# robin-karlsson0/ViT-Adapter

Hardware: AMD Instinct MI355X
Metric: images/sec ViT-Adapter-B 1024x1024 fwd+bwd (+AdamW step) (higher is better)
Workload: dtype bf16; 1 GPU; ViT-Adapter-base_det (det) 1024x1024, per-GPU batch 2, train mode, drop_path 0.3, SyncBN, step = fwd+bwd+AdamW; global_batch=2, parallelism=dp1, hip_graph=True, rccl_ranks=1, gemm_candidates_rejected=0

## Files before the change

vit-adapter_amd/csrc/attn_win.hip:

```cpp
#include "attn_common.h"
#include "common.h"

namespace vah {
namespace attn {
namespace {



template <typename T, int NB, int NT>
__device__ __forceinline__ void stage_rows(const T *const (&src)[NT], const int64_t (&lds)[NT], T *const (&dst)[NT],
                                           const RowMap &rm, int z, int N) {
    vec8<T> x[4][NT];
    bool ok[4];
#pragma unroll
    for (int it = 0; it < 4; ++it) {
        const int i = threadIdx.x + it * 64 * NB;
        const int row = i >> 3, c = (i & 7) * 8;
        const int64_t g = row < N ? grow(rm, z, row, N) : -1;
        ok[it] = g >= 0;
        const int64_t gl = ok[it] ? g : 0;
#pragma unroll
        for (int t = 0; t < NT; ++t) x[it][t] = *reinterpret_cast<const vec8<T> *>(src[t] + gl * lds[t] + c);
    }
#pragma unroll
    for (int it = 0; it < 4; ++it) {
        const int i = threadIdx.x + it * 64 * NB;
        const int row = i >> 3, c = (i & 7) * 8;
#pragma unroll
        for (int t = 0; t < NT; ++t) {
            vec8<T> y = x[it][t];
#pragma unroll
            for (int j = 0; j < 8; ++j) y[j] = ok[it] ? y[j] : (T)0.f;
            *reinterpret_cast<vec8<T> *>(dst[t] + row * kPadRow + c) = y;
        }
    }
}

template <typename T>
__device__ __forceinline__ const T *tile_lane_base(const T *tile, int lane) {
    const int grp = lane >> 4, i16 = lane & 15;
    return tile + (4 * (grp >> 1) + (i16 >> 2)) * kPadRow + 16 * (grp & 1) + 4 * (i16 & 3);
}
template <typename T>
__device__ __forceinline__ vec8<T> load_tr(const T *base, int tok0, int db) {
    const T *p0 = base + tok0 * kPadRow + 32 * db;
    return tr_frag<T>(p0, p0 + 8 * kPadRow);
}

template <typename T, int NB>
__global__ __launch_bounds__(64 * NB) __attribute__((amdgpu_waves_per_eu((2 * NB + 3) / 4, (2 * NB + 3) / 4))) void attn_win_fwd_kernel(
    const T *__restrict__ q, const T *__restrict__ k, const T *__restrict__ v, int64_t ld, RowMap rm,
    int N, int H, float scale_log2, T *__restrict__ out, int64_t ld_out, float *__restrict__ lse) {
    constexpr int ROWS = 32 * NB;
    __shared__ __attribute__((aligned(16))) T s_k[ROWS * kPadRow];
    __shared__ __attribute__((aligned(16))) T s_v[ROWS * kPadRow];
    const int h = blockIdx.x, z = blockIdx.y;
    const int wave = threadIdx.x >> 6, lane = threadIdx.x & 63;
    const int r = lane & 31, hf = lane >> 5;
    const T *qb = q + (int64_t)h * kHD, *kb_ = k + (int64_t)h * kHD, *vb = v + (int64_t)h * kHD;

    const int qrow = wave * 32 + r;
    const int64_t gq = qrow < N ? grow(rm, z, qrow, N) : -1;
    vec8<T> qf[4];
    {
        const int64_t gl = gq >= 0 ? gq : 0;
#pragma unroll
        for (int kk = 0; kk < 4; ++kk) {
            const vec8<T> x = *reinterpret_cast<const vec8<T> *>(qb + gl * ld + 16 * kk + 8 * hf);
#pragma unroll
            for (int j = 0; j < 8; ++j) qf[kk][j] = gq >= 0 ? x[j] : (T)0.f;
        }
    }
    stage_rows<T, NB, 2>({kb_, vb}, {ld, ld}, {s_k, s_v}, rm, z, N);
    __syncthreads();

    auto s_block = [&](int kb) {
        f32x16 s = zero16();
#pragma unroll
        for (int kk = 0; kk < 4; ++kk)
            s = mfma(*reinterpret_cast<const vec8<T> *>(s_k + (kb * 32 + r) * kPadRow + 16 * kk + 8 * hf), qf[kk], s);
        if (kb == NB - 1) {
#pragma unroll
            for (int i = 0; i < 16; ++i)
                if (kb * 32 + crow(i, hf) >= N) s[i] = -INFINITY;
        }
        return s;
    };
    float mx = -INFINITY;
#pragma unroll 1
    for (int kb = 0; kb < NB; ++kb) {
        const f32x16 s = s_block(kb);
#pragma unroll
        for (int i = 0; i < 16; ++i) mx = fmaxf(mx, s[i]);
    }
    mx = fmaxf(mx, __shfl_xor(mx, 32, 64));
    const float m = mx * scale_log2;

    f32x16 o[2] = {zero16(), zero16()};
    float psum = 0.f;
    const T *vbase = tile_lane_base(s_v, lane);
#pragma unroll 1
    for (int kb = 0; kb < NB; ++kb) {
        f32x16 s = s_block(kb);
#pragma unroll
        for (int i = 0; i < 16; ++i) {
            s[i] = __builtin_amdgcn_exp2f(s[i] * scale_log2 - m);
            psum += s[i];
        }
#pragma unroll
        for (int sp = 0; sp < 2; ++sp) {
            const vec8<T> pf = pack_half<T>(s, sp);
#pragma unroll
            for (int db = 0; db < 2; ++db) o[db] = mfma(load_tr(vbase, kb * 32 + 16 * sp, db), pf, o[db]);
        }
    }
    const float l_tot = psum + __shfl_xor(psum, 32, 64);

    const float inv = 1.f / l_tot;
    if (qrow < N && gq >= 0) {
        T *op = out + gq * ld_out + (int64_t)h * kHD;
#pragma unroll
        for (int db = 0; db < 2; ++db)
#pragma unroll
            for (int g = 0; g < 4; ++g) {
                vec4<T> w;
#pragma unroll
                for (int j = 0; j < 4; ++j) w[j] = (T)(o[db][4 * g + j] * inv);
                *reinterpret_cast<vec4<T> *>(op + db * 32 + 8 * g + 4 * hf) = w;
            }
        if (hf == 0) lse[((int64_t)z * H + h) * N + qrow] = m + log2f(l_tot);
    } else if (qrow < N && hf == 0) {
        lse[((int64_t)z * H + h) * N + qrow] = INFINITY;
    }
}


template <typename T, int NB>
__global__ __launch_bounds__(64 * NB) void attn_win_bwd_kernel(
    const T *__restrict__ q, const T *__restrict__ k, const T *__restrict__ v, int64_t ld,
    const T *__restrict__ o, const T *__restrict__ d_o, int64_t ld_out, RowMap rm, const float *__restrict__ lse,
    int N, int H, float scale, float scale_log2, T *__restrict__ dq, T *__restrict__ dk, T *__restrict__ dv,
    int64_t ld_d) {
    constexpr int ROWS = 32 * NB;
    extern __shared__ __attribute__((aligned(16))) unsigned char smem[];
    T *s_q = reinterpret_cast<T *>(smem);
    T *s_k = s_q + ROWS * kPadRow, *s_v = s_k + ROWS * kPadRow, *s_do = s_v + ROWS * kPadRow;
    float *s_lse = reinterpret_cast<float *>(s_do + ROWS * kPadRow), *s_delta = s_lse + ROWS;
    const int h = blockIdx.x, z = blockIdx.y;
    const int wave = threadIdx.x >> 6, lane = threadIdx.x & 63;
    const int r = lane & 31, hf = lane >> 5;
    const int row = wave * 32 + r;
    const int64_t grow_ = row < N ? grow(rm, z, row, N) : -1;
    const bool stored = grow_ >= 0;

    float part = 0.f;
    {
        const int64_t gl = stored ? grow_ : 0;
        const T *op = o + gl * ld_out + (int64_t)h * kHD + 32 * hf, *gp = d_o + gl * ld_out + (int64_t)h * kHD + 32 * hf;
        vec8<T> a[4], b[4];
#pragma unroll
        for (int c = 0; c < 4; ++c) {
            a[c] = *reinterpret_cast<const vec8<T> *>(op + 8 * c);
            b[c] = *reinterpret_cast<const vec8<T> *>(gp + 8 * c);
        }
#pragma unroll
        for (int c = 0; c < 4; ++c)
#pragma unroll
            for (int j = 0; j < 8; ++j) part += (float)a[c][j] * (float)b[c][j];
    }
    const float lse_raw = lse[((int64_t)z * H + h) * N + (row < N ? row : 0)];
    stage_rows<T, NB, 4>({q + (int64_t)h * kHD, k + (int64_t)h * kHD, v + (int64_t)h * kHD, d_o + (int64_t)h * kHD},
                      {ld, ld, ld, ld_out}, {s_q, s_k, s_v, s_do}, rm, z, N);
    const float delta_q = stored ? part + __shfl_xor(part, 32, 64) : 0.f;
    const float lse_q = stored ? lse_raw : INFINITY;
    if (hf == 0) {
        s_lse[row] = lse_q;
        s_delta[row] = delta_q;
    }
    __syncthreads();

    {
        vec8<T> qf[4], dof[4];
#pragma unroll
        for (int kk = 0; kk < 4; ++kk) {
            qf[kk] = *reinterpret_cast<const vec8<T> *>(s_q + row * kPadRow + 16 * kk + 8 * hf);
            dof[kk] = *reinterpret_cast<const vec8<T> *>(s_do + row * kPadRow + 16 * kk + 8 * hf);
        }
        f32x16 acc[2] = {zero16(), zero16()};
        const T *kbase = tile_lane_base(s_k, lane);
#pragma unroll
        for (int j = 0; j < NB; ++j) {
            f32x16 s = zero16(), dp = zero16();
#pragma unroll
            for (int kk = 0; kk < 4; ++kk) {
                const vec8<T> ak = *reinterpret_cast<const vec8<T> *>(s_k + (j * 32 + r) * kPadRow + 16 * kk + 8 * hf);
                const vec8<T> av = *reinterpret_cast<const vec8<T> *>(s_v + (j * 32 + r) * kPadRow + 16 * kk + 8 * hf);
                s = mfma(ak, qf[kk], s);
                dp = mfma(av, dof[kk], dp);
            }
#pragma unroll
            for (int i = 0; i < 16; ++i) s[i] = __builtin_amdgcn_exp2f(s[i] * scale_log2 - lse_q) * (dp[i] - delta_q);
#pragma unroll
            for (int sp = 0; sp < 2; ++sp) {
                const vec8<T> pf = pack_half<T>(s, sp);
#pragma unroll
                for (int db = 0; db < 2; ++db) acc[db] = mfma(load_tr(kbase, j * 32 + 16 * sp, db), pf, acc[db]);
            }
        }
        if (stored) {
            T *op = dq + grow_ * ld_d + (int64_t)h * kHD;
#pragma unroll
            for (int db = 0; db < 2; ++db)
#pragma unroll
                for (int g = 0; g < 4; ++g) {
                    vec4<T> w;
#pragma unroll
                    for (int jj = 0; jj < 4; ++jj) w[jj] = (T)(acc[db][4 * g + jj] * scale);
                    *reinterpret_cast<vec4<T> *>(op + db * 32 + 8 * g + 4 * hf) = w;
                }
        }
    }

    {
        vec8<T> kf[4], vf[4];
#pragma unroll
        for (int kk = 0; kk < 4; ++kk) {
            kf[kk] = *reinterpret_cast<const vec8<T> *>(s_k + row * kPadRow + 16 * kk + 8 * hf);
            vf[kk] = *reinterpret_cast<const vec8<T> *>(s_v + row * kPadRow + 16 * kk + 8 * hf);
        }
        f32x16 dkt[2] = {zero16(), zero16()}, dvt[2] = {zero16(), zero16()};
        const T *qbase = tile_lane_base(s_q, lane), *dobase = tile_lane_base(s_do, lane);
#pragma unroll 1
        for (int i = 0; i < NB; ++i) {
            f32x16 s = zero16(), dp = zero16();
#pragma unroll
            for (int kk = 0; kk < 4; ++kk) {
                const vec8<T> aq = *reinterpret_cast<const vec8<T> *>(s_q + (i * 32 + r) * kPadRow + 16 * kk + 8 * hf);
                const vec8<T> ad = *reinterpret_cast<const vec8<T> *>(s_do + (i * 32 + r) * kPadRow + 16 * kk + 8 * hf);
                s = mfma(aq, kf[kk], s);
                dp = mfma(ad, vf[kk], dp);
            }
#pragma unroll
            for (int g = 0; g < 4; ++g) {
                const float4 l4 = *reinterpret_cast<const float4 *>(s_lse + i * 32 + 8 * g + 4 * hf);
                const float4 d4 = *reinterpret_cast<const float4 *>(s_delta + i * 32 + 8 * g + 4 * hf);
                const float ls[4] = {l4.x, l4.y, l4.z, l4.w}, de[4] = {d4.x, d4.y, d4.z, d4.w};
#pragma unroll
                for (int jj = 0; jj < 4; ++jj) {
                    const int e = 4 * g + jj;
                    const float p = __builtin_amdgcn_exp2f(s[e] * scale_log2 - ls[jj]);
                    s[e] = p;
                    dp[e] = p * (dp[e] - de[jj]);
                }
            }
#pragma unroll
            for (int sp = 0; sp < 2; ++sp) {
                const vec8<T> pf = pack_half<T>(s, sp), dsf = pack_half<T>(dp, sp);
#pragma unroll
                for (int db = 0; db < 2; ++db) {
                    dvt[db] = mfma(load_tr(dobase, i * 32 + 16 * sp, db), pf, dvt[db]);
                    dkt[db] = mfma(load_tr(qbase, i * 32 + 16 * sp, db), dsf, dkt[db]);
                }
            }
        }
        if (stored) {
            T *pk = dk + grow_ * ld_d + (int64_t)h * kHD, *pv = dv + grow_ * ld_d + (int64_t)h * kHD;
#pragma unroll
            for (int db = 0; db < 2; ++db)
#pragma unroll
                for (int g = 0; g < 4; ++g) {
                    vec4<T> wk, wv;
#pragma unroll
                    for (int jj = 0; jj < 4; ++jj) {
                        wk[jj] = (T)(dkt[db][4 * g + jj] * scale);
                        wv[jj] = (T)dvt[db][4 * g + jj];
                    }
                    *reinterpret_cast<vec4<T> *>(pk + db * 32 + 8 * g + 4 * hf) = wk;
                    *reinterpret_cast<vec4<T> *>(pv + db * 32 + 8 * g + 4 * hf) = wv;
                }
        }
    }
}

template <typename T, int NB>
int launch_win_bwd(const T *q, const T *k, const T *v, int64_t ld, const T *o, const T *d_o,
                   int64_t ld_out, RowMap rm, const float *lse, int64_t Z, int64_t H, int N, float scale, T *dq,
                   T *dk, T *dv, int64_t ld_d, hipStream_t st) {
    constexpr int lds = 4 * 32 * NB * kPadRow * 2 + 2 * 32 * NB * 4;
    if (int rc = allow_dynamic_lds((const void *)attn_win_bwd_kernel<T, NB>, lds, "attn_win_bwd")) return rc;
    hipLaunchKernelGGL((attn_win_bwd_kernel<T, NB>), dim3((unsigned)H, (unsigned)Z), dim3(64 * NB), lds, st, q, k, v, ld, o, d_o,
                       ld_out, rm, lse, N, (int)H, scale, scale * 1.4426950408889634f, dq, dk, dv, ld_d);
    return check_launch("attn_win_bwd");
}

template <typename T, int NB>
int launch_win_fwd(const T *q, const T *k, const T *v, int64_t ld, RowMap rm, int64_t Z, int64_t H, int N,
                   float scale_log2, T *out, int64_t ld_out, float *lse, hipStream_t st) {
    hipLaunchKernelGGL((attn_win_fwd_kernel<T, NB>), dim3((unsigned)H, (unsigned)Z), dim3(64 * NB), 0, st, q, k, v, ld, rm, N, (int)H,
                       scale_log2, out, ld_out, lse);
    return check_launch("attn_win_fwd");
}

}

template <typename T>
int attn_win_fwd_resident(const void *q, const void *k, const void *v, int64_t ld, RowMap rm, int64_t Z, int64_t H, int64_t N,
                          float scale, void *out, int64_t ld_out, float *lse, hipStream_t st) {
    if (N < 1 || N > 224 || Z > 65535 || H > 65535) return -1;
    const int NB = (int)((N + 31) / 32);
    const float scale_log2 = scale * 1.4426950408889634f;
#define VAH_CASE(B_)                                                                                                    \
    if (NB == B_)                                                                                                       \
        return launch_win_fwd<T, B_>((const T *)q, (const T *)k, (const T *)v, ld, rm, Z, H, (int)N, scale_log2, \
                                  (T *)out, ld_out, lse, st)
    VAH_CASE(1);
    VAH_CASE(2);
    VAH_CASE(3);
    VAH_CASE(4);
    VAH_CASE(5);
    VAH_CASE(6);
    VAH_CASE(7);
#undef VAH_CASE
    return -1;
}


template <typename T>
int attn_win_bwd_resident(const void *q, const void *k, const void *v, int64_t ld, const void *o, const void *d_o,
                          int64_t ld_out, RowMap rm, const float *lse, int64_t Z, int64_t H, int64_t N, float scale, void *dq,
                          void *dk, void *dv, int64_t ld_d, hipStream_t st) {
    if (N < 1 || N > 224 || Z > 65535 || H > 65535) return -1;
    const int NB = (int)((N + 31) / 32);
#define VAH_CASE(B_)                                                                                                     \
    if (NB == B_)                                                                                                        \
        return launch_win_bwd<T, B_>((const T *)q, (const T *)k, (const T *)v, ld, (const T *)o,         \
                                  (const T *)d_o, ld_out, rm, lse, Z, H, (int)N, scale, (T *)dq, (T *)dk, \
                                  (T *)dv, ld_d, st)
    VAH_CASE(1);
    VAH_CASE(2);
    VAH_CASE(3);
    VAH_CASE(4);
    VAH_CASE(5);
    VAH_CASE(6);
    VAH_CASE(7);
#undef VAH_CASE
    return -1;
}

template int attn_win_fwd_resident<__bf16>(const void *, const void *, const void *, int64_t, RowMap, int64_t, int64_t, int64_t, float,
                                           void *, int64_t, float *, hipStream_t);
template int attn_win_fwd_resident<_Float16>(const void *, const void *, const void *, int64_t, RowMap, int64_t, int64_t, int64_t,
                                             float, void *, int64_t, float *, hipStream_t);
template int attn_win_bwd_resident<__bf16>(const void *, const void *, const void *, int64_t, const void *, const void *, int64_t,
                                           RowMap, const float *, int64_t, int64_t, int64_t, float, void *, void *, void *, int64_t,
                                           hipStream_t);
template int attn_win_bwd_resident<_Float16>(const void *, const void *, const void *, int64_t, const void *, const void *, int64_t,
                                             RowMap, const float *, int64_t, int64_t, int64_t, float, void *, void *, void *, int64_t,
                                             hipStream_t);

}
}
```

Baseline: 77.28 images/sec.

## Skip padded rows in windowed attention via per-window-class item mapping

Flattens the grid to one dimension and maps each block to a (window, head) item grouped by window class: interior, bottom edge, right edge and corner. Each block computes the real row count of its window, exits the waves that only cover padding, and loops over real key blocks only. Padded keys that the original code treated as zero-valued keys are accounted for analytically in the softmax denominator, and padded rows get an infinite LSE. This removes the MFMA and load work spent on padding in edge windows, at the cost of extra index arithmetic per block and more complex masking logic.

```diff
diff --git a/vit-adapter_amd/csrc/attn_win.hip b/vit-adapter_amd/csrc/attn_win.hip
--- a/vit-adapter_amd/csrc/attn_win.hip
+++ b/vit-adapter_amd/csrc/attn_win.hip
@@ -7,31 +7,93 @@
 
 
 
+struct WinItem {
+    int z, h;
+    int vw, Nr, win;
+    int W;
+    int64_t row0;
+    __device__ __forceinline__ int64_t grow(int c) const {
+        const int ly = c / vw;
+        return row0 + (int64_t)ly * W + (c - ly * vw);
+    }
+    __device__ __forceinline__ int local(int c) const {
+        const int ly = c / vw;
+        return ly * win + (c - ly * vw);
+    }
+};
+
+__device__ __forceinline__ WinItem win_item(const RowMap &rm, int item, int H, int Z, int N) {
+    WinItem it;
+    if (rm.win == 0) {
+        it.z = item / H;
+        it.h = item - it.z * H;
+        it.vw = it.Nr = it.win = N;
+        it.W = 0;
+        it.row0 = (int64_t)it.z * N;
+        return it;
+    }
+    const int nwy = rm.nwin / rm.nwx, fy = rm.H / rm.win, fx = rm.W / rm.win, B = Z / rm.nwin;
+    const int cnt[4] = {fy * fx, (nwy - fy) * fx, fy * (rm.nwx - fx), (nwy - fy) * (rm.nwx - fx)};
+    int t = item, cls = 0;
+#pragma unroll
+    for (int c = 0; c < 3; ++c)
+        if (cls == c && t >= B * H * cnt[c]) {
+            t -= B * H * cnt[c];
+            cls = c + 1;
+        }
+    const int u = t / H, per = cnt[cls];
+    it.h = t - u * H;
+    const int b = u / per, j = u - b * per;
+    int wy, wx;
+    if (cls == 0) {
+        wy = j / fx;
+        wx = j - wy * fx;
+    } else if (cls == 1) {
+        wy = fy;
+        wx = j;
+    } else if (cls == 2) {
+        wy = j;
+        wx = fx;
+    } else {
+        wy = fy;
+        wx = fx;
+    }
+    it.z = b * rm.nwin + wy * rm.nwx + wx;
+    const int y0 = wy * rm.win, x0 = wx * rm.win;
+    const int vh = min(rm.win, rm.H - y0);
+    it.vw = min(rm.win, rm.W - x0);
+    it.Nr = vh * it.vw;
+    it.win = rm.win;
+    it.W = rm.W;
+    it.row0 = ((int64_t)b * rm.H + y0) * rm.W + x0;
+    return it;
+}
+
 template <typename T, int NB, int NT>
 __device__ __forceinline__ void stage_rows(const T *const (&src)[NT], const int64_t (&lds)[NT], T *const (&dst)[NT],
-                                           const RowMap &rm, int z, int N) {
+                                           const WinItem &wi, int rows) {
     vec8<T> x[4][NT];
-    bool ok[4];
 #pragma unroll
     for (int it = 0; it < 4; ++it) {
         const int i = threadIdx.x + it * 64 * NB;
         const int row = i >> 3, c = (i & 7) * 8;
-        const int64_t g = row < N ? grow(rm, z, row, N) : -1;
-        ok[it] = g >= 0;
-        const int64_t gl = ok[it] ? g : 0;
-#pragma unroll
-        for (int t = 0; t < NT; ++t) x[it][t] = *reinterpret_cast<const vec8<T> *>(src[t] + gl * lds[t] + c);
+#pragma unroll
+        for (int t = 0; t < NT; ++t)
+#pragma unroll
+            for (int j = 0; j < 8; ++j) x[it][t][j] = (T)0.f;
+        if (row < wi.Nr) {
+            const int64_t g = wi.grow(row);
+#pragma unroll
+            for (int t = 0; t < NT; ++t) x[it][t] = *reinterpret_cast<const vec8<T> *>(src[t] + g * lds[t] + c);
+        }
     }
 #pragma unroll
     for (int it = 0; it < 4; ++it) {
         const int i = threadIdx.x + it * 64 * NB;
         const int row = i >> 3, c = (i & 7) * 8;
-#pragma unroll
-        for (int t = 0; t < NT; ++t) {
-            vec8<T> y = x[it][t];
-#pragma unroll
-            for (int j = 0; j < 8; ++j) y[j] = ok[it] ? y[j] : (T)0.f;
-            *reinterpret_cast<vec8<T> *>(dst[t] + row * kPadRow + c) = y;
+        if (row < rows) {
+#pragma unroll
+            for (int t = 0; t < NT; ++t) *reinterpret_cast<vec8<T> *>(dst[t] + row * kPadRow + c) = x[it][t];
         }
     }
 }
@@ -54,41 +116,50 @@
     constexpr int ROWS = 32 * NB;
     __shared__ __attribute__((aligned(16))) T s_k[ROWS * kPadRow];
     __shared__ __attribute__((aligned(16))) T s_v[ROWS * kPadRow];
-    const int h = blockIdx.x, z = blockIdx.y;
+    const WinItem wi = win_item(rm, blockIdx.x, H, gridDim.x / H, N);
+    const int h = wi.h, z = wi.z, Nr = wi.Nr;
+    const int nb = (Nr + 31) >> 5;
+    const int n_pad = N - Nr;
     const int wave = threadIdx.x >> 6, lane = threadIdx.x & 63;
     const int r = lane & 31, hf = lane >> 5;
     const T *qb = q + (int64_t)h * kHD, *kb_ = k + (int64_t)h * kHD, *vb = v + (int64_t)h * kHD;
+    float *lse_w = lse + ((int64_t)z * H + h) * N;
 
     const int qrow = wave * 32 + r;
-    const int64_t gq = qrow < N ? grow(rm, z, qrow, N) : -1;
+    const bool real_q = qrow < Nr;
+    const int64_t gq = real_q ? wi.grow(qrow) : 0;
     vec8<T> qf[4];
-    {
-        const int64_t gl = gq >= 0 ? gq : 0;
-#pragma unroll
-        for (int kk = 0; kk < 4; ++kk) {
-            const vec8<T> x = *reinterpret_cast<const vec8<T> *>(qb + gl * ld + 16 * kk + 8 * hf);
-#pragma unroll
-            for (int j = 0; j < 8; ++j) qf[kk][j] = gq >= 0 ? x[j] : (T)0.f;
-        }
-    }
-    stage_rows<T, NB, 2>({kb_, vb}, {ld, ld}, {s_k, s_v}, rm, z, N);
+#pragma unroll
+    for (int kk = 0; kk < 4; ++kk) {
+#pragma unroll
+        for (int j = 0; j < 8; ++j) qf[kk][j] = (T)0.f;
+        if (real_q) qf[kk] = *reinterpret_cast<const vec8<T> *>(qb + gq * ld + 16 * kk + 8 * hf);
+    }
+    stage_rows<T, NB, 2>({kb_, vb}, {ld, ld}, {s_k, s_v}, wi, nb * 32);
+    if (n_pad > 0) {
+        for (int i = threadIdx.x; i < N; i += 64 * NB) {
+            const int ly = i / wi.win, lx = i - ly * wi.win;
+            if (lx >= wi.vw || ly * wi.vw >= Nr) lse_w[i] = INFINITY;
+        }
+    }
     __syncthreads();
+    if (wave >= nb) return;
 
     auto s_block = [&](int kb) {
         f32x16 s = zero16();
 #pragma unroll
         for (int kk = 0; kk < 4; ++kk)
             s = mfma(*reinterpret_cast<const vec8<T> *>(s_k + (kb * 32 + r) * kPadRow + 16 * kk + 8 * hf), qf[kk], s);
-        if (kb == NB - 1) {
+        if (kb == nb - 1) {
 #pragma unroll
             for (int i = 0; i < 16; ++i)
-                if (kb * 32 + crow(i, hf) >= N) s[i] = -INFINITY;
+                if (kb * 32 + crow(i, hf) >= Nr) s[i] = -INFINITY;
         }
         return s;
     };
-    float mx = -INFINITY;
+    float mx = n_pad > 0 ? 0.f : -INFINITY;
 #pragma unroll 1
-    for (int kb = 0; kb < NB; ++kb) {
+    for (int kb = 0; kb < nb; ++kb) {
         const f32x16 s = s_block(kb);
 #pragma unroll
         for (int i = 0; i < 16; ++i) mx = fmaxf(mx, s[i]);
@@ -100,7 +171,7 @@
     float psum = 0.f;
     const T *vbase = tile_lane_base(s_v, lane);
 #pragma unroll 1
-    for (int kb = 0; kb < NB; ++kb) {
+    for (int kb = 0; kb < nb; ++kb) {
         f32x16 s = s_block(kb);
 #pragma unroll
         for (int i = 0; i < 16; ++i) {
@@ -114,10 +185,11 @@
             for (int db = 0; db < 2; ++db) o[db] = mfma(load_tr(vbase, kb * 32 + 16 * sp, db), pf, o[db]);
         }
     }
-    const float l_tot = psum + __shfl_xor(psum, 32, 64);
+    float l_tot = psum + __shfl_xor(psum, 32, 64);
+    if (n_pad > 0) l_tot += (float)n_pad * __builtin_amdgcn_exp2f(-m);
 
     const float inv = 1.f / l_tot;
-    if (qrow < N && gq >= 0) {
+    if (real_q) {
         T *op = out + gq * ld_out + (int64_t)h * kHD;
 #pragma unroll
         for (int db = 0; db < 2; ++db)
@@ -128,9 +200,7 @@
                 for (int j = 0; j < 4; ++j) w[j] = (T)(o[db][4 * g + j] * inv);
                 *reinterpret_cast<vec4<T> *>(op + db * 32 + 8 * g + 4 * hf) = w;
             }
-        if (hf == 0) lse[((int64_t)z * H + h) * N + qrow] = m + log2f(l_tot);
-    } else if (qrow < N && hf == 0) {
-        lse[((int64_t)z * H + h) * N + qrow] = INFINITY;
+        if (hf == 0) lse_w[wi.local(qrow)] = m + log2f(l_tot);
     }
 }
 
@@ -146,17 +216,18 @@
     T *s_q = reinterpret_cast<T *>(smem);
     T *s_k = s_q + ROWS * kPadRow, *s_v = s_k + ROWS * kPadRow, *s_do = s_v + ROWS * kPadRow;
     float *s_lse = reinterpret_cast<float *>(s_do + ROWS * kPadRow), *s_delta = s_lse + ROWS;
-    const int h = blockIdx.x, z = blockIdx.y;
+    const WinItem wi = win_item(rm, blockIdx.x, H, gridDim.x / H, N);
+    const int h = wi.h, z = wi.z, Nr = wi.Nr;
+    const int nb = (Nr + 31) >> 5;
     const int wave = threadIdx.x >> 6, lane = threadIdx.x & 63;
     const int r = lane & 31, hf = lane >> 5;
     const int row = wave * 32 + r;
-    const int64_t grow_ = row < N ? grow(rm, z, row, N) : -1;
-    const bool stored = grow_ >= 0;
-
-    float part = 0.f;
-    {
-        const int64_t gl = stored ? grow_ : 0;
-        const T *op = o + gl * ld_out + (int64_t)h * kHD + 32 * hf, *gp = d_o + gl * ld_out + (int64_t)h * kHD + 32 * hf;
+    const bool stored = row < Nr;
+    const int64_t grow_ = stored ? wi.grow(row) : 0;
+
+    float part = 0.f, lse_raw = INFINITY;
+    if (stored) {
+        const T *op = o + grow_ * ld_out + (int64_t)h * kHD + 32 * hf, *gp = d_o + grow_ * ld_out + (int64_t)h * kHD + 32 * hf;
         vec8<T> a[4], b[4];
 #pragma unroll
         for (int c = 0; c < 4; ++c) {
@@ -167,17 +238,18 @@
         for (int c = 0; c < 4; ++c)
 #pragma unroll
             for (int j = 0; j < 8; ++j) part += (float)a[c][j] * (float)b[c][j];
-    }
-    const float lse_raw = lse[((int64_t)z * H + h) * N + (row < N ? row : 0)];
+        lse_raw = lse[((int64_t)z * H + h) * N + wi.local(row)];
+    }
     stage_rows<T, NB, 4>({q + (int64_t)h * kHD, k + (int64_t)h * kHD, v + (int64_t)h * kHD, d_o + (int64_t)h * kHD},
-                      {ld, ld, ld, ld_out}, {s_q, s_k, s_v, s_do}, rm, z, N);
+                      {ld, ld, ld, ld_out}, {s_q, s_k, s_v, s_do}, wi, nb * 32);
     const float delta_q = stored ? part + __shfl_xor(part, 32, 64) : 0.f;
-    const float lse_q = stored ? lse_raw : INFINITY;
+    const float lse_q = lse_raw;
     if (hf == 0) {
         s_lse[row] = lse_q;
         s_delta[row] = delta_q;
     }
     __syncthreads();
+    if (wave >= nb) return;
 
     {
         vec8<T> qf[4], dof[4];
@@ -188,8 +260,8 @@
         }
         f32x16 acc[2] = {zero16(), zero16()};
         const T *kbase = tile_lane_base(s_k, lane);
-#pragma unroll
-        for (int j = 0; j < NB; ++j) {
+#pragma unroll 1
+        for (int j = 0; j < nb; ++j) {
             f32x16 s = zero16(), dp = zero16();
 #pragma unroll
             for (int kk = 0; kk < 4; ++kk) {
@@ -200,6 +272,11 @@
             }
 #pragma unroll
             for (int i = 0; i < 16; ++i) s[i] = __builtin_amdgcn_exp2f(s[i] * scale_log2 - lse_q) * (dp[i] - delta_q);
+            if (j == nb - 1) {
+#pragma unroll
+                for (int i = 0; i < 16; ++i)
+                    if (j * 32 + crow(i, hf) >= Nr) s[i] = 0.f;
+            }
 #pragma unroll
             for (int sp = 0; sp < 2; ++sp) {
                 const vec8<T> pf = pack_half<T>(s, sp);
@@ -231,7 +308,7 @@
         f32x16 dkt[2] = {zero16(), zero16()}, dvt[2] = {zero16(), zero16()};
         const T *qbase = tile_lane_base(s_q, lane), *dobase = tile_lane_base(s_do, lane);
 #pragma unroll 1
-        for (int i = 0; i < NB; ++i) {
+        for (int i = 0; i < nb; ++i) {
             f32x16 s = zero16(), dp = zero16();
 #pragma unroll
             for (int kk = 0; kk < 4; ++kk) {
@@ -288,7 +365,7 @@
                    T *dk, T *dv, int64_t ld_d, hipStream_t st) {
     constexpr int lds = 4 * 32 * NB * kPadRow * 2 + 2 * 32 * NB * 4;
     if (int rc = allow_dynamic_lds((const void *)attn_win_bwd_kernel<T, NB>, lds, "attn_win_bwd")) return rc;
-    hipLaunchKernelGGL((attn_win_bwd_kernel<T, NB>), dim3((unsigned)H, (unsigned)Z), dim3(64 * NB), lds, st, q, k, v, ld, o, d_o,
+    hipLaunchKernelGGL((attn_win_bwd_kernel<T, NB>), dim3((unsigned)(H * Z)), dim3(64 * NB), lds, st, q, k, v, ld, o, d_o,
                        ld_out, rm, lse, N, (int)H, scale, scale * 1.4426950408889634f, dq, dk, dv, ld_d);
     return check_launch("attn_win_bwd");
 }
@@ -296,7 +373,7 @@
 template <typename T, int NB>
 int launch_win_fwd(const T *q, const T *k, const T *v, int64_t ld, RowMap rm, int64_t Z, int64_t H, int N,
                    float scale_log2, T *out, int64_t ld_out, float *lse, hipStream_t st) {
-    hipLaunchKernelGGL((attn_win_fwd_kernel<T, NB>), dim3((unsigned)H, (unsigned)Z), dim3(64 * NB), 0, st, q, k, v, ld, rm, N, (int)H,
+    hipLaunchKernelGGL((attn_win_fwd_kernel<T, NB>), dim3((unsigned)(H * Z)), dim3(64 * NB), 0, st, q, k, v, ld, rm, N, (int)H,
                        scale_log2, out, ld_out, lse);
     return check_launch("attn_win_fwd");
 }
@@ -306,7 +383,7 @@
 template <typename T>
 int attn_win_fwd_resident(const void *q, const void *k, const void *v, int64_t ld, RowMap rm, int64_t Z, int64_t H, int64_t N,
                           float scale, void *out, int64_t ld_out, float *lse, hipStream_t st) {
-    if (N < 1 || N > 224 || Z > 65535 || H > 65535) return -1;
+    if (N < 1 || N > 224 || Z > 65535 || H > 65535 || Z * H > 0x7fffffff) return -1;
     const int NB = (int)((N + 31) / 32);
     const float scale_log2 = scale * 1.4426950408889634f;
 #define VAH_CASE(B_)                                                                                                    \
@@ -329,7 +406,7 @@
 int attn_win_bwd_resident(const void *q, const void *k, const void *v, int64_t ld, const void *o, const void *d_o,
                           int64_t ld_out, RowMap rm, const float *lse, int64_t Z, int64_t H, int64_t N, float scale, void *dq,
                           void *dk, void *dv, int64_t ld_d, hipStream_t st) {
-    if (N < 1 || N > 224 || Z > 65535 || H > 65535) return -1;
+    if (N < 1 || N > 224 || Z > 65535 || H > 65535 || Z * H > 0x7fffffff) return -1;
     const int NB = (int)((N + 31) / 32);
 #define VAH_CASE(B_)                                                                                                     \
     if (NB == B_)                                                                                                        \
```

Measured after the change: 77.65 images/sec, median of 6. No clear change (+0.5%).
